# paganpasta/eqxvision

Measured on AMD Instinct MI355X. Metric: images/sec, higher is better.
Workload: dtype bf16; 1 GPU; resnet50 bf16 forward, batch=256/GPU, 3x224x224, 1000 classes; global_batch=256, parallelism=dp1, graph=True, lanes=2, collective_forced_1rank=False

## Files before the change

### eqxvision_amd/_lib.py

```python
from __future__ import annotations

import ctypes as C
import os
import threading

from . import _trace

_HERE = os.path.dirname(os.path.abspath(__file__))
LIB_PATH = os.environ.get("EQV_LIB") or os.path.join(_HERE, "csrc", "libeqxvision_amd.so")

F32, BF16 = 0, 1
ACT_NONE, ACT_RELU, ACT_GELU_TANH = 0, 1, 2
ACT_HARD_SWISH, ACT_HARD_SIGMOID, ACT_SIGMOID, ACT_SILU = 3, 4, 5, 6
ABI_VERSION = 2

_vp, _i, _f, _i64 = C.c_void_p, C.c_int, C.c_float, C.c_int64

PROTOTYPES = {
    "mv_abi_version": [],
    "mv_last_error": [],
    "mv_last_kernel": [],
    "mv_set_flag": [C.c_char_p, _i],
    "mv_get_flag": [C.c_char_p],
    "mv_flags_epoch": [],
# ... 53 lines not shown
    "mv_cnblock_dw_fwd": [_vp, _vp, _vp, _vp, _i, _i, _i, _i, _f, _i, _i, _i, _vp],
    "mv_conv2d_nchw_split_fwd": [_vp, _vp, _vp, _vp, _vp, _vp] + [_i] * 11 + [_i, _i, _i, _vp],
    "mv_resize_bilinear_nhwc_fwd": [_vp, _vp] + [_i] * 6 + [_i, _i, _i, _vp],
    "mv_copy_rows": [_vp, _vp, _i64, _i64, _i64, _i64, _vp],
    "mv_maxpool2d_nhwc_fwd": [_vp, _vp] + [_i] * 10 + [_i, _vp],
    "mv_adaptive_avgpool2d_nhwc_fwd": [_vp, _vp] + [_i] * 6 + [_i, _i, _vp],
    "mv_layernorm_fwd": [_vp, _vp, _vp, _vp, _i64, _i, _i64, _f, _i, _i, _vp],
    "mv_mha_fwd": [_vp, _vp, _vp, _i, _i, _i, _i, _f, _i, _vp],
    "mv_stem_conv_pool_supported": [_i] * 14 + [_i64],
    "mv_stem_conv_pool_fwd": [_vp, _vp, _vp, _vp, _vp] + [_i] * 17 + [_vp],
    "mv_conv1x1_chain_supported": [_i64, _i, _i, _i, _i],
    "mv_conv1x1_chain_fwd": [_vp] * 10 + [_i64, _i, _i, _i, _i, _vp],
    "mv_bottleneck_tail_supported": [_i] * 5,
    "mv_bottleneck_tail_fwd": [_vp] * 9 + [_i] * 6 + [_vp],
    "mv_conv1x1_dual_supported": [_i64, _i, _i, _i, _i],
    "mv_conv1x1_dual_fwd": [_vp] * 6 + [_i] * 11 + [_vp],
    "mv_conv1x1_chain_res_supported": [_i] * 8,
    "mv_conv1x1_chain_res_fwd": [_vp] * 6 + [_i] * 8 + [_vp],
    "mv_conv1x1_chain_rc_supported": [_i64, _i, _i, _i, _i],
    "mv_conv1x1_chain_rc_fwd": [_vp] * 7 + [_i64, _i, _i, _i, _i, _vp],
    "mv_conv1x1_chain_rc0_fwd": [_vp] * 5 + [_i64, _i, _i, _i, _i, _vp],
    "mv_conv1x1_chain_sub_supported": [_i] * 7,
    "mv_conv1x1_chain_sub_fwd": [_vp] * 10 + [_i] * 7 + [_vp],
    "mv_conv1x1_dual_chain_supported": [_i64, _i, _i, _i, _i, _i],
    "mv_conv1x1_dual_chain_fwd": [_vp] * 10 + [_i64, _i, _i, _i, _i, _i, _vp],
    "mv_linear_heads_supported": [_i64, _i, _i, _i, _i, _i],
    "mv_linear_lnout_supported": [_i64, _i, _i, _i],
    "mv_linear_lnout_fwd": [_vp, _vp, _vp, _vp, _vp, _vp, _vp, _vp, _i64, _i, _i, _i, _vp],
    "mv_linear_lnin_supported": [_i64, _i, _i, _i, _i, _i],
    "mv_linear_lnin_fwd": [_vp, _vp, _vp, _vp, _vp, _vp, _i64, _i, _i, _f, _i, _i, _i, _i, _vp],
    "mv_linear_heads_fwd": [_vp, _vp, _vp, _vp, _vp, _i64, _i, _i, _i, _i, _i, _vp],
    "mv_mha_heads_fwd": [_vp, _vp, _vp, _i, _i, _i, _i, _f, _i, _vp],
    "mv_mha_dropout_fwd": [_vp, _i, _vp, _vp, _vp, _f, _i, _i, _i, _i, _f, _i, _vp],
    "mv_swin_window_attn_fwd": [_vp, _vp, _vp] + [_i] * 9 + [_i, _vp],
    "mv_patch_merge_gather_nhwc": [_vp, _vp, _i, _i, _i, _i, _i, _vp],
    "mv_patch4_ln_supported": [_i] * 5,
    "mv_patch4_ln_fwd": [_vp] * 7 + [_i] * 5 + [_f, _i, _vp],
    "mv_patch_merge_ln_supported": [_i] * 4,
    "mv_patch_merge_ln_fwd": [_vp, _vp, _vp, _vp, _i, _i, _i, _i, _f, _i, _i, _vp],
    "mv_vit_cls_pos_fwd": [_vp, _vp, _vp, _i, _i, _i, _i, _vp],
    "mv_eltwise_fwd": [_vp, _vp, _i64, _i, _i, _vp],
    "mv_add_fwd": [_vp, _vp, _vp, _i64, _i, _i, _vp],
    "mv_channel_affine_fwd": [_vp, _vp, _vp, _vp, _i64, _i, _i, _i, _vp],
    "mv_channel_affine_res_fwd": [_vp, _vp, _vp, _vp, _vp, _i64, _i, _i, _i, _vp],
    "mv_nchw_to_nhwc": [_vp, _vp, _i, _i, _i, _i, _i, _i, _vp],
    "mv_nhwc_to_nchw": [_vp, _vp, _i, _i, _i, _i, _i, _i, _vp],
# ... 153 lines not shown
```

### eqxvision_amd/csrc/chain_rc.hip

```cpp
#include "mfma_common.h"

namespace mv {

struct ChainRcP {
    const bf16_t* t2;
    const bf16_t* t2p;
    const bf16_t* x0;
    const bf16_t* wf;
    const unsigned* sh;
    bf16_t* y;
    bf16_t* t1;
    int M, tiles_m;
    int dbg;
};

typedef short s16x2 __attribute__((ext_vector_type(2)));
__device__ __forceinline__ uint32_t relu_pack_bf2(float a, float b) {
    uint32_t w = pack_bf2(a, b);
    asm volatile("" : "+v"(w));
    const s16x2 z = {0, 0};
    return __builtin_bit_cast(uint32_t, __builtin_elementwise_max(__builtin_bit_cast(s16x2, w), z));
}

template <int NPREV, int WAVES, int RD>
__global__ __launch_bounds__(WAVES * 64) void chain_rc_kernel(const ChainRcP p) {
    constexpr int K = 256, N2 = 64, FPC = 12 + 4 * NPREV, NFRAG = 8 * FPC, PITCH = 144, NSH = 8 * (1 + NPREV) + 2, NT = WAVES * 64,
                  NX = 8 + 4 * NPREV;
    extern __shared__ __attribute__((aligned(16))) char smem[];
    char* wl = smem;
    const int tid = threadIdx.x, lane = tid & 63, wave = tid >> 6;
    char* ep = smem + NFRAG * 1024 + NSH * 256 + wave * (32 * PITCH);

    {
        constexpr int N16 = NFRAG * 64, U = 4;
        for (int base = 0; base < N16; base += U * NT) {
            uint4 v[U];
#pragma unroll
            for (int u = 0; u < U; ++u) {
                const int i = base + u * NT + tid;
                v[u] = ((const uint4*)p.wf)[i < N16 ? i : N16 - 1];
            }
#pragma unroll
            for (int u = 0; u < U; ++u) {
                const int i = base + u * NT + tid;
                if (i < N16) ((uint4*)wl)[i] = v[u];
// ... 472 lines not shown
```

### eqxvision_amd/csrc/common.h

```cpp
#pragma once
#include <atomic>
#include <hip/hip_runtime.h>
#include <stdint.h>
#include <stdio.h>
#include <string.h>

#include "../../include/eqxvision_amd.h"

namespace mv {

typedef uint16_t bf16_t;

__device__ __forceinline__ float bf2f(bf16_t v) { return __uint_as_float(((uint32_t)v) << 16); }

typedef __bf16 bf16x2_t __attribute__((ext_vector_type(2)));
__device__ __forceinline__ bf16_t f2bf(float f) { return __builtin_bit_cast(bf16_t, (__bf16)f); }
__device__ __forceinline__ uint32_t pack_bf2(float lo, float hi) {
    bf16x2_t v;
    v[0] = (__bf16)lo;
    v[1] = (__bf16)hi;
    return __builtin_bit_cast(uint32_t, v);
}

template <typename T> struct io;
// ... 134 lines not shown
                  int dh, int dw, int act, int out_dtype, int m_end, int tok, hipStream_t stream);
int igemm2_tile_shape(long long M, int K, int* bm, int* bn);
int igemm2_dual_supported(long long M, int C1, int C2, int K, int dtype);
int igemm2_dual_launch(const void* x, const void* x2, const void* w, const float* scale, const float* shift, void* y, int N,
                       int Ho, int Wo, int C1, int H2, int W2, int C2, int s2, int K, int act, hipStream_t st);
void igemm2_force_tile(int tile);
int tile_override(const char* kind, long long M, int a, int b, int R, int S, int sh);
int chain1x1_supported(long long M, int C, int K, int N2, int dtype);
int chain1x1_dual_supported(long long M, int C1, int C2, int K, int N2, int dtype);
int chain1x1_dual_launch(const void* x, const void* x2, const void* wcat, const float* scale3, const float* shift3, void* y,
                         const void* w1, const float* scale1, const float* shift1, void* t1, long long M, hipStream_t st);
int chain1x1_launch(const void* x, const void* w3, const float* scale3, const float* shift3, const void* residual, void* y,
                    const void* w1, const float* scale1, const float* shift1, void* t1, long long M, int N2, hipStream_t st);
int chain1x1_sub_supported(long long N, int H, int W, int C, int K, int N2, int dtype);
int chain1x1_sub_launch(const void* x, const void* w3, const float* scale3, const float* shift3, const void* residual, void* y_sub,
                        const void* w1, const float* scale1, const float* shift1, void* t1, int N, int H, int W, hipStream_t st);
int chain_rc_supported(long long M, int C, int K, int N2, int dtype);
int chain_rc_launch(const void* t2, const void* t2_prev, const void* x0, const void* wfrag, const void* shifts, void* y, void* t1,
                    long long M, hipStream_t st);
int chain_rc0_launch(const void* t2, const void* x0, const void* wfrag, const void* shifts, void* t1, long long M, hipStream_t st);
int chain_res_supported(long long N, int H, int W, int C, int K, int N2, int sub, int dtype);
int chain_res_launch(const void* t2, const void* residual, const void* wfrag, const void* shifts, void* y, void* t1, int N, int H, int W,
                     int sub, hipStream_t st);
int chain_stream_supported(long long M, int C, int K, int N2, int dtype);
int chain_stream_launch(const void* x, const void* w3, const float* scale3, const float* shift3, const void* residual, void* y,
                        const void* w1, const float* scale1, const float* shift1, void* t1, long long M, hipStream_t st);
int igemm8_supported(long long M, int C, int K, int R, int S, long long x_bytes, long long w_bytes);
int device_status(int clear, unsigned* out);
int igemm8_wanted(long long M, int C, int K, int R, int S);
int igemm8_launch(const void* x, const void* w, const float* scale, const float* shift, const void* residual, void* y,
                  int N, int H, int W, int C, int K, int R, int S, int sh, int sw, int ph, int pw, int dh, int dw,
                  int act, int out_dtype, int tok, int tile, hipStream_t st);
bool igemm8_ln_supported(long long M, int N, int K);
int igemm8_lnout_launch(const void* x, const void* w, const float* shift, const void* res, const void* res_lo, void* y, void* y_lo,
                        float* stats, long long M, int N, int K, hipStream_t st);
int igemm8_lnin_launch(const void* x, const float* stats, const void* w, const float* colsum, const float* shift, void* y, long long M,
                       int N, int K, float eps, int act, int tok, hipStream_t st);
int igemm8_dual_launch(const void* x, const void* x2, const void* w, const float* scale, const float* shift,
                       const void* residual, void* y, int N, int Ho, int Wo, int C1, int H2, int W2, int C2, int s2, int K,
                       int act, int out_dtype, int tile, hipStream_t st);
int stem_supported(int C, int K, int R, int S, int x_dtype, int out_dtype);
int stem_f32out_supported(int C, int H, int W, int K, int R, int S, int sh, int sw, int ph, int pw, int x_dtype);
int stem_launch(const void* x, const void* w, const float* scale, const float* shift, void* y, int N, int C,
                int H, int W, int K, int R, int S, int sh, int sw, int ph, int pw, int act, int x_dtype,
                int out_dtype, int tok_stride, int tok_offset, const float* pos, hipStream_t stream,
                const void* w_lo = nullptr);
// ... 21 lines not shown
```

### eqxvision_amd/csrc/generic.hip

```cpp
#include "mfma_common.h"

namespace mv {

struct ConvP {
    int N, H, W, C, K, R, S, Ho, Wo, sh, sw, ph, pw, dh, dw, groups;
    long long sxn, sxc, sxh, sxw;
    long long swk, swc, swr, sws;
    int act, tok_stride, tok_offset;
};

template <typename TX, typename TW, typename TY>
__global__ void conv_generic_kernel(const TX* __restrict__ x, const TW* __restrict__ w,
                                    const float* __restrict__ scale, const float* __restrict__ shift,
                                    const TY* __restrict__ residual, TY* __restrict__ y,
                                    const float* __restrict__ pos, ConvP p) {
    const int k = blockIdx.y * blockDim.x + threadIdx.x;
    const long long m = (long long)blockIdx.x * blockDim.y + threadIdx.y;
    const long long M = (long long)p.N * p.Ho * p.Wo;
    if (k >= p.K || m >= M) return;
    const int wo = (int)(m % p.Wo);
    const int ho = (int)((m / p.Wo) % p.Ho);
    const int n = (int)(m / ((long long)p.Wo * p.Ho));
    const int Cg = p.C / p.groups, Kg = p.K / p.groups;
    const int g = k / Kg;
// ... 1217 lines not shown
    if (chain_stream_supported(M, C, K, N2, dtype))
        return chain_stream_launch(x, w3, scale3, shift3, residual, y, w1, scale1, shift1, t1, M, (hipStream_t)stream);
    return chain1x1_launch(x, w3, scale3, shift3, residual, y, w1, scale1, shift1, t1, M, N2, (hipStream_t)stream);
}

int mv_conv1x1_chain_sub_supported(int N, int H, int W, int C, int K, int N2, int dtype) {
    return !get_flag("force_generic") && !get_flag("no_stream") && N > 0 && H > 0 && W > 0 && chain1x1_sub_supported(N, H, W, C, K, N2, dtype);
}

int mv_conv1x1_chain_sub_fwd(const void* x, const void* w3, const float* scale3, const float* shift3, const void* residual,
                             void* y_sub, const void* w1, const float* scale1, const float* shift1, void* t1, int N, int H, int W,
                             int C, int K, int N2, int dtype, mv_stream_t stream) {
    MV_CHECK_ARG(x && w3 && residual && y_sub && w1 && t1, "conv1x1_chain_sub: NULL pointer");
    if (!mv_conv1x1_chain_sub_supported(N, H, W, C, K, N2, dtype)) {
        set_error("conv1x1_chain_sub: unsupported shape N=%d H=%d W=%d C=%d K=%d N2=%d (ask mv_conv1x1_chain_sub_supported first)", N, H,
                  W, C, K, N2);
        return MV_E_UNSUPPORTED;
    }
    MV_CHECK_ARG(y_sub != residual && y_sub != x && t1 != y_sub, "conv1x1_chain_sub: y_sub must not alias x / residual / t1");
    return chain1x1_sub_launch(x, w3, scale3, shift3, residual, y_sub, w1, scale1, shift1, t1, N, H, W, (hipStream_t)stream);
}

int mv_conv1x1_chain_res_supported(int N, int H, int W, int C, int K, int N2, int sub, int dtype) {
    return !get_flag("force_generic") && !get_flag("no_stream") && N > 0 && H > 0 && W > 0 && chain_res_supported(N, H, W, C, K, N2, sub, dtype);
}

int mv_conv1x1_chain_res_fwd(const void* t2, const void* residual, const void* wfrag, const void* shifts, void* y, void* t1, int N, int H,
                             int W, int C, int K, int N2, int sub, int dtype, mv_stream_t stream) {
    MV_CHECK_ARG(t2 && residual && wfrag && shifts && y && t1, "conv1x1_chain_res: NULL pointer");
    if (!mv_conv1x1_chain_res_supported(N, H, W, C, K, N2, sub, dtype)) {
        set_error("conv1x1_chain_res: unsupported shape N=%d H=%d W=%d C=%d K=%d N2=%d sub=%d (ask mv_conv1x1_chain_res_supported first)", N,
                  H, W, C, K, N2, sub);
        return MV_E_UNSUPPORTED;
    }
    MV_CHECK_ARG(y != residual && y != t2 && t1 != y && t1 != residual && t1 != t2, "conv1x1_chain_res: outputs must not alias inputs");
    return chain_res_launch(t2, residual, wfrag, shifts, y, t1, N, H, W, sub, (hipStream_t)stream);
}

int mv_conv1x1_chain_rc_supported(int64_t M, int C, int K, int N2, int dtype) {
    return !get_flag("force_generic") && !get_flag("no_stream") && chain_rc_supported(M, C, K, N2, dtype);
}

int mv_conv1x1_chain_rc_fwd(const void* t2, const void* t2_prev, const void* x0, const void* wfrag, const void* shifts, void* y,
                            void* t1, int64_t M, int C, int K, int N2, int dtype, mv_stream_t stream) {
    MV_CHECK_ARG(t2 && t2_prev && x0 && wfrag && shifts && y && t1, "conv1x1_chain_rc: NULL pointer");
    if (!mv_conv1x1_chain_rc_supported(M, C, K, N2, dtype)) {
        set_error("conv1x1_chain_rc: unsupported shape M=%lld C=%d K=%d N2=%d (ask mv_conv1x1_chain_rc_supported first)", (long long)M, C,
                  K, N2);
        return MV_E_UNSUPPORTED;
    }
    MV_CHECK_ARG(y != t2 && y != t2_prev && y != x0 && t1 != y && t1 != t2 && t1 != t2_prev && t1 != x0,
                 "conv1x1_chain_rc: outputs must not alias inputs");
    return chain_rc_launch(t2, t2_prev, x0, wfrag, shifts, y, t1, M, (hipStream_t)stream);
}

int mv_conv1x1_chain_rc0_fwd(const void* t2, const void* x0, const void* wfrag, const void* shifts, void* t1, int64_t M, int C, int K,
                             int N2, int dtype, mv_stream_t stream) {
    MV_CHECK_ARG(t2 && x0 && wfrag && shifts && t1, "conv1x1_chain_rc0: NULL pointer");
    if (!mv_conv1x1_chain_rc_supported(M, C, K, N2, dtype)) {
// ... 752 lines not shown
```

### eqxvision_amd/csrc/mfma_common.h

```cpp
#pragma once
#include "common.h"

namespace mv {

typedef __bf16 bf16x8 __attribute__((ext_vector_type(8)));
typedef float f32x16 __attribute__((ext_vector_type(16)));

__device__ __forceinline__ void glds16(const void* gsrc, void* lds_dst) {
    __builtin_amdgcn_global_load_lds((const __attribute__((address_space(1))) void*)gsrc,
                                     (__attribute__((address_space(3))) void*)lds_dst, 16, 0, 0);
}

__device__ __forceinline__ void wave_lds_fence() {
    __builtin_amdgcn_fence(__ATOMIC_RELEASE, "wavefront");
    __builtin_amdgcn_wave_barrier();
    __builtin_amdgcn_fence(__ATOMIC_ACQUIRE, "wavefront");
}

typedef __amdgpu_buffer_rsrc_t brsrc_t;
typedef unsigned int u32x4_t __attribute__((ext_vector_type(4)));
constexpr unsigned BUF_OOB = 0x80000000u;

__device__ __forceinline__ brsrc_t make_brsrc(const void* base, bool live = true) {
    return __builtin_amdgcn_make_buffer_rsrc((void*)base, (short)0, live ? (int)BUF_OOB : 0, 0x00020000);
}
__device__ __forceinline__ float4 buf_load_f4(brsrc_t r, unsigned vo, unsigned so = 0) {
    const u32x4_t u = __builtin_amdgcn_raw_buffer_load_b128(r, vo, so, 0);
    return make_float4(__uint_as_float(u[0]), __uint_as_float(u[1]), __uint_as_float(u[2]), __uint_as_float(u[3]));
}
__device__ __forceinline__ void buf_store_f4(brsrc_t r, unsigned vo, float4 v) {
    u32x4_t u;
    u[0] = __float_as_uint(v.x); u[1] = __float_as_uint(v.y); u[2] = __float_as_uint(v.z); u[3] = __float_as_uint(v.w);
    __builtin_amdgcn_raw_buffer_store_b128(u, r, vo, 0, 0);
}
__device__ __forceinline__ uint4 buf_load_u4(brsrc_t r, unsigned vo, unsigned so = 0) {
    const u32x4_t u = __builtin_amdgcn_raw_buffer_load_b128(r, vo, so, 0);
    return make_uint4(u[0], u[1], u[2], u[3]);
}
__device__ __forceinline__ void buf_store_u4(brsrc_t r, unsigned vo, uint4 v) {
// ... 83 lines not shown
```

### eqxvision_amd/ops.py

```python
from __future__ import annotations

from typing import Optional, Tuple

import numpy as np
import torch

from . import _lib
from ._act import (Act, is_act, DT, TORCH_DT, compute_dtype, device, empty, head_fp32, on_replay, residual_fp32, split_weights,
                   stream_ptr)

ACT = {None: _lib.ACT_NONE, "none": _lib.ACT_NONE, "relu": _lib.ACT_RELU, "gelu": _lib.ACT_GELU_TANH,
       "hard_swish": _lib.ACT_HARD_SWISH, "hard_sigmoid": _lib.ACT_HARD_SIGMOID, "sigmoid": _lib.ACT_SIGMOID, "silu": _lib.ACT_SILU}
UNFUSED_ACTS = ("hard_swish", "hard_sigmoid", "sigmoid", "silu")


def _ptr(t: Optional[torch.Tensor]):
    return None if t is None else t.data_ptr()


def _dev(a: np.ndarray, dtype: torch.dtype) -> torch.Tensor:
    a = np.ascontiguousarray(a)
    if dtype == torch.bfloat16 and a.dtype == np.float32 and a.size < (1 << 20):
        u = a.view(np.uint32)
        r = ((u >> np.uint32(16)) & np.uint32(1)) + np.uint32(0x7FFF)
# ... 356 lines not shown
    y = empty((B, Ho, Wo, K), torch.bfloat16)
    _lib.call("mv_copy_rows", _ptr(yp), _ptr(y), B * Ho * Wo, K * 2, Kp * 2, K * 2, stream_ptr())
    return Act(y, "map", x.batched)


def _pointwise(conv) -> bool:
    return (tuple(conv.kernel_size) == (1, 1) and tuple(conv.stride) == (1, 1) and tuple(conv.padding) == (0, 0)
            and tuple(conv.dilation) == (1, 1) and conv.groups == 1)


def conv1x1_chain(x: Act, conv3, bn3, residual: Act, conv1n, bn1n, sub: int = 0) -> Optional[Act]:
    dt = compute_dtype()
    if dt != "bf16" or not (_pointwise(conv3) and _pointwise(conv1n)) or conv3.out_channels != conv1n.in_channels:
        return None
    if _bn_training(bn3) or _bn_training(bn1n):
        return None
    x, residual = as_map(x), as_map(residual)
    B, H, W, C = x.t.shape
    K, N2 = conv3.out_channels, conv1n.out_channels
    M = B * H * W
    if C != conv3.in_channels or tuple(residual.t.shape) != (B, H, W, K) or x.t.dtype != torch.bfloat16 \
            or residual.t.dtype != torch.bfloat16:
        return None
    if not _lib.load().mv_conv1x1_chain_supported(M, C, K, N2, DT[dt]):
        return None
    lib = _lib.load()
    for sb in ((2, 0) if sub == 2 else (0,)):
        if lib.mv_conv1x1_chain_res_supported(B, H, W, C, K, N2, sb, DT[dt]):
            wf, shf, _ = chain_res_fragments(conv3, bn3, conv1n, bn1n)
            y = empty((B, H // 2, W // 2, K) if sb else (B, H, W, K), torch.bfloat16)
            t1 = empty((B, H, W, N2), torch.bfloat16)
            _lib.call("mv_conv1x1_chain_res_fwd", _ptr(x.t), _ptr(residual.t), _ptr(wf), _ptr(shf), _ptr(y), _ptr(t1), B, H, W, C, K, N2,
                      sb, DT[dt], stream_ptr())
            out = Act(y, "map", x.batched)
            out.sub = 2 if sb else None
            out.pre = (conv1n, Act(t1, "map", x.batched))
            return out
    w3, s3, h3 = prep_conv(conv3, bn3, "krsc", dt)
    w1, s1, h1 = prep_conv(conv1n, bn1n, "krsc", dt)
    t1 = empty((B, H, W, N2), torch.bfloat16)
    if sub == 2 and _lib.load().mv_conv1x1_chain_sub_supported(B, H, W, C, K, N2, DT[dt]):
        y = empty((B, H // 2, W // 2, K), torch.bfloat16)
        _lib.call("mv_conv1x1_chain_sub_fwd", _ptr(x.t), _ptr(w3), _ptr(s3), _ptr(h3), _ptr(residual.t), _ptr(y), _ptr(w1), _ptr(s1),
                  _ptr(h1), _ptr(t1), B, H, W, C, K, N2, DT[dt], stream_ptr())
        out = Act(y, "map", x.batched)
        out.sub = 2
    else:
        y = empty((B, H, W, K), torch.bfloat16)
        _lib.call("mv_conv1x1_chain_fwd", _ptr(x.t), _ptr(w3), _ptr(s3), _ptr(h3), _ptr(residual.t), _ptr(y), _ptr(w1), _ptr(s1),
                  _ptr(h1), _ptr(t1), M, C, K, N2, DT[dt], stream_ptr())
        out = Act(y, "map", x.batched)
    out.pre = (conv1n, Act(t1, "map", x.batched))
    return out


def _rc_shift_rows(*vecs) -> np.ndarray:
    rows = []
    for v in vecs:
        v = np.asarray(v, np.float32).reshape(-1, 32)
        hi = torch.from_numpy(v).to(torch.bfloat16)
# ... 27 lines not shown
        frags = np.empty((K // 32, 16, 2, 32, 8), np.float32)
        e8 = np.arange(8)
        for c in range(K // 32):
            rows = slice(32 * c, 32 * c + 32)
            for fh in range(2):
                for kk in range(8):
                    frags[c, kk, fh] = wcat[rows][:, 16 * kk + 8 * fh + e8]
                for kk in range(4):
                    frags[c, 8 + kk, fh] = w31[rows][:, 16 * kk + 8 * fh + e8]
            _rc_conv1n_frags(frags, 12, w1n, c)
        sh = _rc_shift_rows(h30 + hd, h1, hn)
        hit = (_dev(frags.reshape(-1), torch.bfloat16), torch.from_numpy(sh.view(np.int32)).to(device()), (conv3_0, ds_conv, conv1n))
        cache[key] = hit
    return hit


def chain_res_fragments(conv3, bn3, conv1n, bn1n):
    cache = conv3._cache()
    key = ("chain_res", _bn_id(bn3), id(conv1n), _bn_id(bn1n))
    hit = cache.get(key)
    if hit is None:
        w3, h3 = _scaled_rows(conv3, bn3)
        w1n, hn = _scaled_rows(conv1n, bn1n)
        K, T2 = w3.shape[0], w1n.shape[0] // 32
        frags = np.empty((K // 32, 4 + 2 * T2, 2, 32, 8), np.float32)
        e8 = np.arange(8)
        for c in range(K // 32):
            rows = slice(32 * c, 32 * c + 32)
            for fh in range(2):
                for kk in range(4):
                    frags[c, kk, fh] = w3[rows][:, 16 * kk + 8 * fh + e8]
                for s_ in range(2):
                    cols = 32 * c + 16 * s_ + 4 * fh + np.array([0, 1, 2, 3, 8, 9, 10, 11])
                    for a2 in range(T2):
                        frags[c, 4 + T2 * s_ + a2, fh] = w1n[32 * a2:32 * a2 + 32][:, cols]
        sh = _rc_shift_rows(h3, hn)
        hit = (_dev(frags.reshape(-1), torch.bfloat16), torch.from_numpy(sh.view(np.int32)).to(device()), conv1n)
        cache[key] = hit
    return hit


def chain_rc0_fragments(conv3_0, bn3_0, ds_conv, ds_bn, conv1n, bn1n):
    cache = conv3_0._cache()
    key = ("chain_rc0", _bn_id(bn3_0), id(ds_conv), _bn_id(ds_bn), id(conv1n), _bn_id(bn1n))
    hit = cache.get(key)
    if hit is None:
        w30, h30 = _scaled_rows(conv3_0, bn3_0)
        wd, hd = _scaled_rows(ds_conv, ds_bn)
        wcat = np.concatenate([w30, wd], axis=1)
        w1n, hn = _scaled_rows(conv1n, bn1n)
        K = wcat.shape[0]
        frags = np.empty((K // 32, 12, 2, 32, 8), np.float32)
        e8 = np.arange(8)
        for c in range(K // 32):
            rows = slice(32 * c, 32 * c + 32)
            for fh in range(2):
                for kk in range(8):
                    frags[c, kk, fh] = wcat[rows][:, 16 * kk + 8 * fh + e8]
            _rc_conv1n_frags(frags, 8, w1n, c)
        sh = _rc_shift_rows(h30 + hd, hn)
# ... 142 lines not shown


def chain_rc_available(x: Act, b0, cd, b1, b2) -> bool:
    if compute_dtype() != "bf16" or _lib.get_flag("no_chain_rc"):
        return False
    convs = (b0.conv3, cd[0], b1.conv1, b1.conv3, b2.conv1)
    if not all(_pointwise(c) for c in convs) or any(_bn_training(b) for b in (b0.bn1, b0.bn2, b0.bn3, cd[1], b1.bn1, b1.bn2, b1.bn3, b2.bn1)):
        return False
    if x.kind != "map" or x.t.dtype != torch.bfloat16:
        return False
    B, H, W, C = x.t.shape
    M, K = B * H * W, b0.conv3.out_channels
    if b0.conv3.in_channels != C or cd[0].in_channels != C or b1.conv3.in_channels != C or cd[0].out_channels != K \
            or b1.conv3.out_channels != K or b1.conv1.in_channels != K or b2.conv1.in_channels != K \
            or tuple(b0.conv2.stride) != (1, 1) or tuple(b1.conv2.stride) != (1, 1) or b0.conv2.out_channels != C or b1.conv2.out_channels != C:
        return False
    lib = _lib.load()
    return bool(lib.mv_conv1x1_dual_chain_supported(M, C, C, K, b1.conv1.out_channels, DT["bf16"])
                and lib.mv_conv1x1_chain_rc_supported(M, C, K, b2.conv1.out_channels, DT["bf16"]))


def conv1x1_dual_chain(x: Act, conv3, bn3, xin: Act, ds_conv, ds_bn, conv1n, bn1n, store_y: bool = True) -> Optional[Act]:
    dt = compute_dtype()
    if dt != "bf16" or not (_pointwise(conv3) and _pointwise(ds_conv) and _pointwise(conv1n)):
        return None
    if conv3.out_channels != ds_conv.out_channels or conv3.out_channels != conv1n.in_channels:
        return None
    if any(_bn_training(b) for b in (bn3, ds_bn, bn1n)):
        return None
    x, xin = as_map(x), as_map(xin)
    B, H, W, C1 = x.t.shape
    C2, K, N2 = xin.t.shape[-1], conv3.out_channels, conv1n.out_channels
    M = B * H * W
    if tuple(xin.t.shape[:3]) != (B, H, W) or C1 != conv3.in_channels or C2 != ds_conv.in_channels \
            or x.t.dtype != torch.bfloat16 or xin.t.dtype != torch.bfloat16:
        return None
    if not _lib.load().mv_conv1x1_dual_chain_supported(M, C1, C2, K, N2, DT[dt]):
        return None
    if not store_y and not _lib.get_flag("no_chain_rc0") and _lib.load().mv_conv1x1_chain_rc_supported(M, C1, K, N2, DT[dt]):
        wf, tab, _ = chain_rc0_fragments(conv3, bn3, ds_conv, ds_bn, conv1n, bn1n)
        t1 = empty((B, H, W, N2), torch.bfloat16)
        _lib.call("mv_conv1x1_chain_rc0_fwd", _ptr(x.t), _ptr(xin.t), _ptr(wf), _ptr(tab), _ptr(t1), M, C1, K, N2, DT[dt], stream_ptr())
        return Act(t1, "map", x.batched)
    wcat, shift = _dual_weights(conv3, bn3, ds_conv, ds_bn)
    w1, s1, h1 = prep_conv(conv1n, bn1n, "krsc", dt)
    y = empty((B, H, W, K), torch.bfloat16) if store_y else None
    t1 = empty((B, H, W, N2), torch.bfloat16)
    _lib.call("mv_conv1x1_dual_chain_fwd", _ptr(x.t), _ptr(xin.t), _ptr(wcat), None, _ptr(shift), _ptr(y), _ptr(w1), _ptr(s1),
              _ptr(h1), _ptr(t1), M, C1, C2, K, N2, DT[dt], stream_ptr())
    if not store_y:
        return Act(t1, "map", x.batched)
    out = Act(y, "map", x.batched)
    out.pre = (conv1n, Act(t1, "map", x.batched))
    return out


def stem_conv_pool(x: Act, conv, bn, act, pool) -> Act:
    if _bn_training(bn):
        return maxpool2d(conv2d(x, conv, bn, act), pool.kernel_size, pool.stride, pool.padding)
    dt = compute_dtype()
# ... 953 lines not shown
```

### include/eqxvision_amd.h

```cpp
#ifndef EQXVISION_AMD_H
#define EQXVISION_AMD_H

#include <stddef.h>
#include <stdint.h>

#ifdef __cplusplus
extern "C" {
#endif

#define MV_ABI_VERSION 2

typedef void* mv_stream_t;

enum { MV_F32 = 0, MV_BF16 = 1 };
enum { MV_ACT_NONE = 0, MV_ACT_RELU = 1, MV_ACT_GELU_TANH = 2, MV_ACT_HARD_SWISH = 3, MV_ACT_HARD_SIGMOID = 4, MV_ACT_SIGMOID = 5,
       MV_ACT_SILU = 6 };
enum { MV_OK = 0, MV_E_INVALID = -1, MV_E_UNSUPPORTED = -2, MV_E_OOM = -3 };

int mv_abi_version(void);
const char* mv_last_error(void);
int mv_set_flag(const char* name, int value);
int mv_get_flag(const char* name);
int mv_flags_epoch(void);
int mv_device_status(int clear, unsigned* status);
// ... 28 lines not shown
                         const void* residual, void* y, const void* w1, const float* scale1,
                         const float* shift1, void* t1, int64_t M, int C, int K, int N2, int dtype,
                         mv_stream_t stream);

int mv_bottleneck_tail_supported(int H, int W, int width, int cout, int dtype);
int mv_bottleneck_tail_fwd(const void* t1, const void* w2f, const float* scale2, const float* shift2, const void* w3f,
                           const float* scale3, const float* shift3, const void* residual, void* y, int B, int H, int W,
                           int width, int cout, int dtype, mv_stream_t stream);

int mv_conv1x1_dual_supported(int64_t M, int C1, int C2, int K, int dtype);
int mv_conv1x1_dual_fwd(const void* x, const void* x2, const void* wcat, const float* scale, const float* shift,
                        void* y, int N, int Ho, int Wo, int C1, int H2, int W2, int C2, int stride2, int K,
                        int act, int dtype, mv_stream_t stream);

int mv_conv1x1_dual_chain_supported(int64_t M, int C1, int C2, int K, int N2, int dtype);
int mv_conv1x1_dual_chain_fwd(const void* x, const void* x2, const void* wcat, const float* scale,
                              const float* shift, void* y, const void* w1, const float* scale1,
                              const float* shift1, void* t1, int64_t M, int C1, int C2, int K, int N2,
                              int dtype, mv_stream_t stream);

int mv_conv1x1_chain_res_supported(int N, int H, int W, int C, int K, int N2, int sub, int dtype);
int mv_conv1x1_chain_res_fwd(const void* t2, const void* residual, const void* wfrag, const void* shifts, void* y, void* t1, int N, int H,
                             int W, int C, int K, int N2, int sub, int dtype, mv_stream_t stream);
int mv_conv1x1_chain_rc_supported(int64_t M, int C, int K, int N2, int dtype);
int mv_conv1x1_chain_rc0_fwd(const void* t2, const void* x0, const void* wfrag, const void* shifts, void* t1, int64_t M, int C, int K,
                             int N2, int dtype, mv_stream_t stream);
int mv_conv1x1_chain_rc_fwd(const void* t2, const void* t2_prev, const void* x0, const void* wfrag, const void* shifts, void* y,
                            void* t1, int64_t M, int C, int K, int N2, int dtype, mv_stream_t stream);
int mv_conv1x1_chain_sub_supported(int N, int H, int W, int C, int K, int N2, int dtype);
int mv_conv1x1_chain_sub_fwd(const void* x, const void* w3, const float* scale3, const float* shift3, const void* residual,
                             void* y_sub, const void* w1, const float* scale1, const float* shift1, void* t1, int N, int H, int W,
                             int C, int K, int N2, int dtype, mv_stream_t stream);

int mv_linear_fwd(const void* x, const void* w, const float* scale, const float* shift,
                  const void* residual, void* y, int64_t M, int N, int K,
                  int act, int in_dtype, int out_dtype, mv_stream_t stream);

int mv_linear_split_supported(int64_t M, int N, int K, int dtype);
int mv_linear_split_fwd(const void* x, const void* w_hi_lo, const float* scale, const float* shift, const void* residual,
                        void* y, int64_t M, int N, int K, int act, int in_dtype, int out_dtype, mv_stream_t stream);
int mv_conv2d_nchw_split_fwd(const void* x, const void* w_hi, const void* w_lo, const float* scale, const float* shift,
                             void* y, int N, int C, int H, int W, int K, int R, int S, int sh, int sw, int ph, int pw,
                             int act, int x_dtype, int out_dtype, mv_stream_t stream);

int mv_channel_scale_nhwc_fwd(const void* x, const void* s, void* y, int N, int64_t HW, int C, int dtype, mv_stream_t stream);

// ... 197 lines not shown
```

Baseline: 84690 images/s.

## Add fused layer2 chain kernels for residual and dual-downsample bottleneck transitions

```diff
diff --git a/eqxvision_amd/_lib.py b/eqxvision_amd/_lib.py
--- a/eqxvision_amd/_lib.py
+++ b/eqxvision_amd/_lib.py
@@ -99,6 +99,8 @@
     "mv_conv1x1_chain_rc0_fwd": [_vp] * 5 + [_i64, _i, _i, _i, _i, _vp],
     "mv_conv1x1_chain_sub_supported": [_i] * 7,
     "mv_conv1x1_chain_sub_fwd": [_vp] * 10 + [_i] * 7 + [_vp],
+    "mv_conv1x1_dual_chain_res_supported": [_i64, _i, _i, _i, _i, _i],
+    "mv_conv1x1_dual_chain_res_fwd": [_vp] * 6 + [_i64, _i, _i, _i, _i, _i, _vp],
     "mv_conv1x1_dual_chain_supported": [_i64, _i, _i, _i, _i, _i],
     "mv_conv1x1_dual_chain_fwd": [_vp] * 10 + [_i64, _i, _i, _i, _i, _i, _vp],
     "mv_linear_heads_supported": [_i64, _i, _i, _i, _i, _i],
diff --git a/eqxvision_amd/csrc/chain_l2.hip b/eqxvision_amd/csrc/chain_l2.hip
--- /dev/null
+++ b/eqxvision_amd/csrc/chain_l2.hip
@@ -0,0 +1,312 @@
+#include <type_traits>
+#include "mfma_common.h"
+
+namespace mv {
+
+struct ChainL2P {
+    const bf16_t* xa;
+    const bf16_t* xb;
+    const bf16_t* res;
+    const bf16_t* wf;
+    const unsigned* sh;
+    bf16_t* y;
+    bf16_t* t1;
+    int M, tiles_m, subH, subW, rounds, act;
+};
+
+template <int C1, int C2, bool RES, int N2, bool SUB, int WAVES, int AHEAD, int RD>
+__global__ __launch_bounds__(WAVES * 64) void chain_l2_kernel(const ChainL2P p) {
+    constexpr int K = 512, NCH = K / 32, KA = C1 / 16, KX = (C1 + C2) / 16, T2 = N2 / 32, FPC = KX + 2 * T2, CB = FPC * 1024,
+                  NSH = NCH + T2, NT = WAVES * 64, PT = FPC * 64 / NT, PITCH = 144;
+    static_assert((FPC * 64) % NT == 0 && RD <= FPC && (AHEAD == 1 || AHEAD == 2) && NCH % 2 == 0, "chain_l2 shape");
+    extern __shared__ __attribute__((aligned(16))) char smem[];
+    char* wbuf = smem;
+    unsigned* shl = (unsigned*)(smem + 2 * CB);
+    const int tid = threadIdx.x, lane = tid & 63, wave = tid >> 6;
+    char* ep = smem + 2 * CB + NSH * 256 + wave * (32 * PITCH);
+
+    auto wload = [&](int c, u32x4_t* wr) {
+        const u32x4_t* src = (const u32x4_t*)p.wf + c * (CB / 16);
+#pragma unroll
+        for (int u = 0; u < PT; ++u) wr[u] = src[u * NT + tid];
+    };
+    auto wstore = [&](int buf, const u32x4_t* wr) {
+#pragma unroll
+        for (int u = 0; u < PT; ++u) ((u32x4_t*)(wbuf + buf * CB))[u * NT + tid] = wr[u];
+    };
+    auto block_sync = [&]() {
+        asm volatile("s_waitcnt lgkmcnt(0)\n\ts_barrier" ::: "memory");
+        __builtin_amdgcn_sched_barrier(0);
+    };
+
+    u32x4_t wreg[AHEAD][PT];
+    wload(0, wreg[0]);
+    if constexpr (AHEAD == 2) wload(1, wreg[1]);
+    for (int i = tid; i < NSH * 64; i += NT) shl[i] = p.sh[i];
+    wstore(0, wreg[0]);
+    block_sync();
+
+    const int fr = lane & 31, fh = lane >> 5;
+    typedef __attribute__((address_space(3))) const char* lds_cp;
+    unsigned wb0 = (unsigned)(uintptr_t)(lds_cp)wbuf + lane * 16;
+    unsigned wb1 = wb0 + CB;
+    unsigned sbase = (unsigned)(uintptr_t)(lds_cp)(const char*)shl + lane * 4;
+    asm volatile("" : "+v"(wb0), "+v"(wb1), "+v"(sbase));
+    auto afrag = [&](int buf, int f) -> bf16x8 {
+        const lds_cp b = (lds_cp)(uintptr_t)(buf ? wb1 : wb0);
+        return __builtin_bit_cast(bf16x8, *(const __attribute__((address_space(3))) u32x4_t*)(b + f * 1024));
+    };
+    auto sfrag = [&](int row) -> bf16x8 {
+        u32x4_t v;
+        v[0] = *(const __attribute__((address_space(3))) unsigned*)((lds_cp)(uintptr_t)sbase + row * 256);
+        v[1] = 0u; v[2] = 0u; v[3] = 0u;
+        return __builtin_bit_cast(bf16x8, v);
+    };
+    u32x4_t onesv;
+    onesv[0] = fh ? 0u : 0x3f803f80u; onesv[1] = 0u; onesv[2] = 0u; onesv[3] = 0u;
+    const bf16x8 ones = __builtin_bit_cast(bf16x8, onesv);
+
+    auto load_x = [&](uint4* xf, int tile) {
+        int m = tile * 32 + fr;
+        m = m < p.M ? m : p.M - 1;
+#pragma unroll
+        for (int kk = 0; kk < KA; ++kk) xf[kk] = *(const uint4*)(p.xa + (long long)m * C1 + fh * 8 + kk * 16);
+#pragma unroll
+        for (int kk = 0; kk < KX - KA; ++kk) xf[KA + kk] = *(const uint4*)(p.xb + (long long)m * C2 + fh * 8 + kk * 16);
+    };
+    struct Rows2 { uint4 r0, r1; };
+    auto load_res = [&](int tile, int c) -> Rows2 {
+        Rows2 o;
+        if constexpr (RES) {
+            auto row = [&](int pass) -> uint4 {
+                int m = tile * 32 + pass * 16 + (lane >> 2);
+                m = m < p.M ? m : p.M - 1;
+                return *(const uint4*)(p.res + (long long)m * K + c * 32 + (lane & 3) * 8);
+            };
+            o.r0 = row(0); o.r1 = row(1);
+        } else {
+            o.r0 = make_uint4(0, 0, 0, 0); o.r1 = o.r0;
+        }
+        return o;
+    };
+
+    uint4 xf[KX];
+    const int tbase = p.tiles_m / (int)gridDim.x, trem = p.tiles_m % (int)gridDim.x;
+    const int nb = tbase + ((int)blockIdx.x < trem ? 1 : 0);
+    const int tile0 = (int)blockIdx.x * tbase + ((int)blockIdx.x < trem ? (int)blockIdx.x : trem);
+    const int wv = __builtin_amdgcn_readfirstlane(wave);
+    int tile = tile0 + wave;
+    load_x(xf, tile);
+    Rows2 rr = load_res(tile, 0);
+
+    for (int r = 0; r < p.rounds; ++r, tile += p.act) {
+        if (!(wv < p.act && r * p.act + wv < nb)) {
+#pragma unroll 1
+            for (int c0 = 0; c0 < NCH; c0 += 2)
+#pragma unroll
+                for (int ci = 0; ci < 2; ++ci) {
+                    const int c = c0 + ci, cn = c + AHEAD < NCH ? c + AHEAD : c + AHEAD - NCH;
+                    wload(cn, wreg[ci % AHEAD]);
+                    wstore(ci ^ 1, wreg[(ci + 1) % AHEAD]);
+                    block_sync();
+                }
+            continue;
+        }
+        const int tile_u = __builtin_amdgcn_readfirstlane(tile);
+        const int ntile = tile + p.act;
+        const brsrc_t ry = SUB ? make_brsrc(p.y) : make_brsrc(p.y + (long long)tile_u * 32 * K);
+        const brsrc_t rt = make_brsrc(p.t1 + (long long)tile_u * 32 * N2);
+        const int rows_left = p.M - tile_u * 32;
+        unsigned yoff[2];
+#pragma unroll
+        for (int pass = 0; pass < 2; ++pass) {
+            const int row = pass * 16 + (lane >> 2);
+            if constexpr (SUB) {
+                const int m = tile_u * 32 + row, hw = p.subH * p.subW;
+                const int b = m / hw, rem = m - b * hw;
+                const int h = rem / p.subW, w = rem - h * p.subW;
+                yoff[pass] = m < p.M && !((h | w) & 1) ? (unsigned)(((b * (p.subH >> 1) + (h >> 1)) * (p.subW >> 1) + (w >> 1)) * K) * 2u
+                                                       : BUF_OOB;
+            } else {
+                yoff[pass] = row < rows_left ? (unsigned)(row * K) * 2u : BUF_OOB;
+            }
+        }
+        f32x16 acc2[T2];
+#pragma unroll
+        for (int a2 = 0; a2 < T2; ++a2) {
+            f32x16 z;
+#pragma unroll
+            for (int e = 0; e < 16; ++e) z[e] = 0.f;
+            acc2[a2] = __builtin_amdgcn_mfma_f32_32x32x16_bf16(sfrag(NCH + a2), ones, z, 0, 0, 0);
+        }
+
+        auto step = [&](auto CI, const int c, auto LAST) {
+            constexpr int ci = decltype(CI)::value;
+            {
+                const int cn = c + AHEAD < NCH ? c + AHEAD : c + AHEAD - NCH;
+                wload(cn, wreg[ci % AHEAD]);
+            }
+            bf16x8 ring[RD];
+#pragma unroll
+            for (int d = 0; d < RD; ++d) ring[d] = afrag(ci, d);
+            auto take = [&](int i) -> bf16x8 {
+                __builtin_amdgcn_sched_barrier(0);
+                const bf16x8 a = ring[i % RD];
+                if (i + RD < FPC) ring[i % RD] = afrag(ci, i + RD);
+                return a;
+            };
+            f32x16 a;
+            if constexpr (RES) {
+                {
+                    char* w = ep + (lane >> 2) * PITCH + (lane & 3) * 16;
+                    *(uint4*)(w) = rr.r0; *(uint4*)(w + 16 * PITCH) = rr.r1;
+                }
+                wave_lds_fence();
+                rr = load_res(c + 1 < NCH ? tile : ntile, c + 1 < NCH ? c + 1 : 0);
+#pragma unroll
+                for (int g = 0; g < 4; ++g) {
+                    const uint2 u = *(const uint2*)(ep + fr * PITCH + (8 * g + 4 * fh) * 2);
+                    a[4 * g] = __uint_as_float(u.x << 16);
+                    a[4 * g + 1] = __uint_as_float(u.x & 0xffff0000u);
+                    a[4 * g + 2] = __uint_as_float(u.y << 16);
+                    a[4 * g + 3] = __uint_as_float(u.y & 0xffff0000u);
+                }
+                wave_lds_fence();
+            } else {
+#pragma unroll
+                for (int e = 0; e < 16; ++e) a[e] = 0.f;
+            }
+            a = __builtin_amdgcn_mfma_f32_32x32x16_bf16(sfrag(c), ones, a, 0, 0, 0);
+#pragma unroll
+            for (int kk = 0; kk < KX; ++kk) {
+                const bf16x8 af = take(kk);
+                a = __builtin_amdgcn_mfma_f32_32x32x16_bf16(af, __builtin_bit_cast(bf16x8, xf[kk]), a, 0, 0, 0);
+                __builtin_amdgcn_sched_barrier(0);
+            }
+            uint32_t pk[8];
+#pragma unroll
+            for (int g = 0; g < 4; ++g) {
+                pk[2 * g] = relu_pack_bf2(a[4 * g], a[4 * g + 1]);
+                pk[2 * g + 1] = relu_pack_bf2(a[4 * g + 2], a[4 * g + 3]);
+                *(uint2*)(ep + fr * PITCH + (8 * g + 4 * fh) * 2) = make_uint2(pk[2 * g], pk[2 * g + 1]);
+            }
+            if constexpr (decltype(LAST)::value) load_x(xf, ntile);
+#pragma unroll
+            for (int q = 0; q < 2 * T2; ++q) {
+                const bf16x8 af = take(KX + q);
+                const int s = q / T2, a2 = q % T2;
+                const uint4 b = make_uint4(pk[4 * s], pk[4 * s + 1], pk[4 * s + 2], pk[4 * s + 3]);
+                acc2[a2] = __builtin_amdgcn_mfma_f32_32x32x16_bf16(af, __builtin_bit_cast(bf16x8, b), acc2[a2], 0, 0, 0);
+                __builtin_amdgcn_sched_barrier(0);
+            }
+            wave_lds_fence();
+#pragma unroll
+            for (int pass = 0; pass < 2; ++pass) {
+                const int row = pass * 16 + (lane >> 2);
+                const uint4 u = *(const uint4*)(ep + row * PITCH + (lane & 3) * 16);
+                buf_store_u4(ry, yoff[pass] == BUF_OOB ? BUF_OOB : yoff[pass] + (unsigned)(c * 32 + (lane & 3) * 8) * 2u, u);
+            }
+            wave_lds_fence();
+            wstore(ci ^ 1, wreg[(ci + 1) % AHEAD]);
+            block_sync();
+        };
+#pragma unroll 1
+        for (int c0 = 0; c0 < NCH - 2; c0 += 2) {
+            step(std::integral_constant<int, 0>(), c0, std::false_type());
+            step(std::integral_constant<int, 1>(), c0 + 1, std::false_type());
+        }
+        step(std::integral_constant<int, 0>(), NCH - 2, std::false_type());
+        step(std::integral_constant<int, 1>(), NCH - 1, std::true_type());
+
+#pragma unroll
+        for (int rd = 0; rd < T2 / 2; ++rd) {
+#pragma unroll
+            for (int a2 = 0; a2 < 2; ++a2)
+#pragma unroll
+                for (int g = 0; g < 4; ++g)
+                    *(uint2*)(ep + fr * PITCH + (a2 * 32 + 8 * g + 4 * fh) * 2) =
+                        make_uint2(relu_pack_bf2(acc2[2 * rd + a2][4 * g], acc2[2 * rd + a2][4 * g + 1]),
+                                   relu_pack_bf2(acc2[2 * rd + a2][4 * g + 2], acc2[2 * rd + a2][4 * g + 3]));
+            wave_lds_fence();
+#pragma unroll
+            for (int pass = 0; pass < 4; ++pass) {
+                const int row = pass * 8 + (lane >> 3);
+                const uint4 u = *(const uint4*)(ep + row * PITCH + (lane & 7) * 16);
+                buf_store_u4(rt, row < rows_left ? (unsigned)(row * N2 + rd * 64 + (lane & 7) * 8) * 2u : BUF_OOB, u);
+            }
+            wave_lds_fence();
+        }
+    }
+}
+
+template <int C1, int C2, bool RES, int N2, bool SUB, int WAVES, int AHEAD, int RD>
+static int chain_l2_go(ChainL2P& p, long long M, hipStream_t st) {
+    constexpr int FPC = (C1 + C2) / 16 + N2 / 16;
+    constexpr int SMEM = 2 * FPC * 1024 + (16 + N2 / 32) * 256 + WAVES * 32 * 144;
+    static_assert(SMEM <= 160 * 1024, "LDS");
+    p.M = (int)M;
+    p.tiles_m = (int)((M + 31) / 32);
+    int gx = 256;
+    const int need = (p.tiles_m + WAVES - 1) / WAVES;
+    if (gx > need) gx = need;
+    const int per_block = (p.tiles_m + gx - 1) / gx;
+    p.rounds = (per_block + WAVES - 1) / WAVES;
+    p.act = (per_block + p.rounds - 1) / p.rounds;
+    auto kern = chain_l2_kernel<C1, C2, RES, N2, SUB, WAVES, AHEAD, RD>;
+    static LdsAttrSite attr;
+    MV_HIP(attr.ensure((const void*)kern, SMEM));
+    hipLaunchKernelGGL(kern, dim3(gx), dim3(WAVES * 64), SMEM, st, p);
+    MV_LAUNCH_CHECK();
+    return MV_OK;
+}
+
+static bool chain_l2_m_ok(long long M) { return M >= 16384 && M < (1LL << 31) - (1 << 20); }
+
+int chain_l2_res_supported(long long N, int H, int W, int C, int K, int N2, int sub, int dtype) {
+    const long long M = N * H * W;
+    if (!(dtype == MV_BF16 && C == 128 && K == 512 && (N2 == 128 || N2 == 256) && chain_l2_m_ok(M)) || get_flag("no_chain") ||
+        get_flag("no_chain_res") || get_flag("no_chain_l2"))
+        return 0;
+    if (sub == 0) return 1;
+    return sub == 2 && H % 2 == 0 && W % 2 == 0 && N * (H / 2) * (W / 2) * K * 2 < (1LL << 31) && !get_flag("no_chain_sub");
+}
+
+int chain_l2_res_launch(const void* t2, const void* residual, const void* wfrag, const void* shifts, void* y, void* t1, int N, int H,
+                        int W, int N2, int sub, hipStream_t st) {
+    ChainL2P p;
+    p.xa = (const bf16_t*)t2; p.xb = nullptr; p.res = (const bf16_t*)residual; p.wf = (const bf16_t*)wfrag;
+    p.sh = (const unsigned*)shifts; p.y = (bf16_t*)y; p.t1 = (bf16_t*)t1;
+    p.subH = H; p.subW = W;
+    const long long M = (long long)N * H * W;
+    if (N2 == 256) {
+        if (sub) {
+            set_kernel_name("chain_l2_exit_bf16_128_512_256_ysub2");
+            return chain_l2_go<128, 0, true, 256, true, 4, 2, 6>(p, M, st);
+        }
+        set_kernel_name("chain_l2_exit_bf16_128_512_256");
+        return chain_l2_go<128, 0, true, 256, false, 4, 2, 6>(p, M, st);
+    }
+    if (sub) {
+        set_kernel_name("chain_l2_res_bf16_128_512_128_ysub2");
+        return chain_l2_go<128, 0, true, 128, true, 8, 2, 6>(p, M, st);
+    }
+    set_kernel_name("chain_l2_res_bf16_128_512_128");
+    return chain_l2_go<128, 0, true, 128, false, 8, 2, 6>(p, M, st);
+}
+
+int chain_l2_dual_supported(long long M, int C1, int C2, int K, int N2, int dtype) {
+    return dtype == MV_BF16 && C1 == 128 && C2 == 256 && K == 512 && N2 == 128 && chain_l2_m_ok(M) && !get_flag("no_chain") &&
+           !get_flag("no_chain_l2");
+}
+
+int chain_l2_dual_launch(const void* t2, const void* x, const void* wfrag, const void* shifts, void* y, void* t1, long long M,
+                         hipStream_t st) {
+    ChainL2P p;
+    p.xa = (const bf16_t*)t2; p.xb = (const bf16_t*)x; p.res = nullptr; p.wf = (const bf16_t*)wfrag;
+    p.sh = (const unsigned*)shifts; p.y = (bf16_t*)y; p.t1 = (bf16_t*)t1;
+    p.subH = 0; p.subW = 0;
+    set_kernel_name("chain_l2_entry_bf16_128+256_512_128");
+    return chain_l2_go<128, 256, false, 128, false, 4, 2, 6>(p, M, st);
+}
+
+}
diff --git a/eqxvision_amd/csrc/chain_rc.hip b/eqxvision_amd/csrc/chain_rc.hip
--- a/eqxvision_amd/csrc/chain_rc.hip
+++ b/eqxvision_amd/csrc/chain_rc.hip
@@ -13,14 +13,6 @@
     int M, tiles_m;
     int dbg;
 };
-
-typedef short s16x2 __attribute__((ext_vector_type(2)));
-__device__ __forceinline__ uint32_t relu_pack_bf2(float a, float b) {
-    uint32_t w = pack_bf2(a, b);
-    asm volatile("" : "+v"(w));
-    const s16x2 z = {0, 0};
-    return __builtin_bit_cast(uint32_t, __builtin_elementwise_max(__builtin_bit_cast(s16x2, w), z));
-}
 
 template <int NPREV, int WAVES, int RD>
 __global__ __launch_bounds__(WAVES * 64) void chain_rc_kernel(const ChainRcP p) {
diff --git a/eqxvision_amd/csrc/common.h b/eqxvision_amd/csrc/common.h
--- a/eqxvision_amd/csrc/common.h
+++ b/eqxvision_amd/csrc/common.h
@@ -180,6 +180,12 @@
 int chain_res_supported(long long N, int H, int W, int C, int K, int N2, int sub, int dtype);
 int chain_res_launch(const void* t2, const void* residual, const void* wfrag, const void* shifts, void* y, void* t1, int N, int H, int W,
                      int sub, hipStream_t st);
+int chain_l2_res_supported(long long N, int H, int W, int C, int K, int N2, int sub, int dtype);
+int chain_l2_res_launch(const void* t2, const void* residual, const void* wfrag, const void* shifts, void* y, void* t1, int N, int H,
+                        int W, int N2, int sub, hipStream_t st);
+int chain_l2_dual_supported(long long M, int C1, int C2, int K, int N2, int dtype);
+int chain_l2_dual_launch(const void* t2, const void* x, const void* wfrag, const void* shifts, void* y, void* t1, long long M,
+                         hipStream_t st);
 int chain_stream_supported(long long M, int C, int K, int N2, int dtype);
 int chain_stream_launch(const void* x, const void* w3, const float* scale3, const float* shift3, const void* residual, void* y,
                         const void* w1, const float* scale1, const float* shift1, void* t1, long long M, hipStream_t st);
diff --git a/eqxvision_amd/csrc/generic.hip b/eqxvision_amd/csrc/generic.hip
--- a/eqxvision_amd/csrc/generic.hip
+++ b/eqxvision_amd/csrc/generic.hip
@@ -1263,7 +1263,8 @@
 }
 
 int mv_conv1x1_chain_res_supported(int N, int H, int W, int C, int K, int N2, int sub, int dtype) {
-    return !get_flag("force_generic") && !get_flag("no_stream") && N > 0 && H > 0 && W > 0 && chain_res_supported(N, H, W, C, K, N2, sub, dtype);
+    return !get_flag("force_generic") && !get_flag("no_stream") && N > 0 && H > 0 && W > 0 &&
+           (chain_res_supported(N, H, W, C, K, N2, sub, dtype) || chain_l2_res_supported(N, H, W, C, K, N2, sub, dtype));
 }
 
 int mv_conv1x1_chain_res_fwd(const void* t2, const void* residual, const void* wfrag, const void* shifts, void* y, void* t1, int N, int H,
@@ -1275,7 +1276,25 @@
         return MV_E_UNSUPPORTED;
     }
     MV_CHECK_ARG(y != residual && y != t2 && t1 != y && t1 != residual && t1 != t2, "conv1x1_chain_res: outputs must not alias inputs");
+    if (C == 128)
+        return chain_l2_res_launch(t2, residual, wfrag, shifts, y, t1, N, H, W, N2, sub, (hipStream_t)stream);
     return chain_res_launch(t2, residual, wfrag, shifts, y, t1, N, H, W, sub, (hipStream_t)stream);
+}
+
+int mv_conv1x1_dual_chain_res_supported(int64_t M, int C1, int C2, int K, int N2, int dtype) {
+    return !get_flag("force_generic") && !get_flag("no_stream") && chain_l2_dual_supported(M, C1, C2, K, N2, dtype);
+}
+
+int mv_conv1x1_dual_chain_res_fwd(const void* t2, const void* x, const void* wfrag, const void* shifts, void* y, void* t1, int64_t M,
+                                  int C1, int C2, int K, int N2, int dtype, mv_stream_t stream) {
+    MV_CHECK_ARG(t2 && x && wfrag && shifts && y && t1, "conv1x1_dual_chain_res: NULL pointer");
+    if (!mv_conv1x1_dual_chain_res_supported(M, C1, C2, K, N2, dtype)) {
+        set_error("conv1x1_dual_chain_res: unsupported shape M=%lld C1=%d C2=%d K=%d N2=%d (ask mv_conv1x1_dual_chain_res_supported first)",
+                  (long long)M, C1, C2, K, N2);
+        return MV_E_UNSUPPORTED;
+    }
+    MV_CHECK_ARG(y != t2 && y != x && t1 != y && t1 != t2 && t1 != x, "conv1x1_dual_chain_res: outputs must not alias inputs");
+    return chain_l2_dual_launch(t2, x, wfrag, shifts, y, t1, M, (hipStream_t)stream);
 }
 
 int mv_conv1x1_chain_rc_supported(int64_t M, int C, int K, int N2, int dtype) {
diff --git a/eqxvision_amd/csrc/mfma_common.h b/eqxvision_amd/csrc/mfma_common.h
--- a/eqxvision_amd/csrc/mfma_common.h
+++ b/eqxvision_amd/csrc/mfma_common.h
@@ -15,6 +15,14 @@
     __builtin_amdgcn_fence(__ATOMIC_RELEASE, "wavefront");
     __builtin_amdgcn_wave_barrier();
     __builtin_amdgcn_fence(__ATOMIC_ACQUIRE, "wavefront");
+}
+
+typedef short s16x2 __attribute__((ext_vector_type(2)));
+__device__ __forceinline__ uint32_t relu_pack_bf2(float a, float b) {
+    uint32_t w = pack_bf2(a, b);
+    asm volatile("" : "+v"(w));
+    const s16x2 z = {0, 0};
+    return __builtin_bit_cast(uint32_t, __builtin_elementwise_max(__builtin_bit_cast(s16x2, w), z));
 }
 
 typedef __amdgpu_buffer_rsrc_t brsrc_t;
diff --git a/eqxvision_amd/ops.py b/eqxvision_amd/ops.py
--- a/eqxvision_amd/ops.py
+++ b/eqxvision_amd/ops.py
@@ -402,8 +402,6 @@
     if C != conv3.in_channels or tuple(residual.t.shape) != (B, H, W, K) or x.t.dtype != torch.bfloat16 \
             or residual.t.dtype != torch.bfloat16:
         return None
-    if not _lib.load().mv_conv1x1_chain_supported(M, C, K, N2, DT[dt]):
-        return None
     lib = _lib.load()
     for sb in ((2, 0) if sub == 2 else (0,)):
         if lib.mv_conv1x1_chain_res_supported(B, H, W, C, K, N2, sb, DT[dt]):
@@ -416,6 +414,8 @@
             out.sub = 2 if sb else None
             out.pre = (conv1n, Act(t1, "map", x.batched))
             return out
+    if not lib.mv_conv1x1_chain_supported(M, C, K, N2, DT[dt]):
+        return None
     w3, s3, h3 = prep_conv(conv3, bn3, "krsc", dt)
     w1, s1, h1 = prep_conv(conv1n, bn1n, "krsc", dt)
     t1 = empty((B, H, W, N2), torch.bfloat16)
@@ -489,20 +489,39 @@
     if hit is None:
         w3, h3 = _scaled_rows(conv3, bn3)
         w1n, hn = _scaled_rows(conv1n, bn1n)
-        K, T2 = w3.shape[0], w1n.shape[0] // 32
-        frags = np.empty((K // 32, 4 + 2 * T2, 2, 32, 8), np.float32)
-        e8 = np.arange(8)
-        for c in range(K // 32):
-            rows = slice(32 * c, 32 * c + 32)
-            for fh in range(2):
-                for kk in range(4):
-                    frags[c, kk, fh] = w3[rows][:, 16 * kk + 8 * fh + e8]
-                for s_ in range(2):
-                    cols = 32 * c + 16 * s_ + 4 * fh + np.array([0, 1, 2, 3, 8, 9, 10, 11])
-                    for a2 in range(T2):
-                        frags[c, 4 + T2 * s_ + a2, fh] = w1n[32 * a2:32 * a2 + 32][:, cols]
         sh = _rc_shift_rows(h3, hn)
-        hit = (_dev(frags.reshape(-1), torch.bfloat16), torch.from_numpy(sh.view(np.int32)).to(device()), conv1n)
+        hit = (_dev(_res_fragments(w3, w1n).reshape(-1), torch.bfloat16), torch.from_numpy(sh.view(np.int32)).to(device()), conv1n)
+        cache[key] = hit
+    return hit
+
+
+def _res_fragments(w3, w1n) -> np.ndarray:
+    K, KX, T2 = w3.shape[0], w3.shape[1] // 16, w1n.shape[0] // 32
+    frags = np.empty((K // 32, KX + 2 * T2, 2, 32, 8), np.float32)
+    e8 = np.arange(8)
+    for c in range(K // 32):
+        rows = slice(32 * c, 32 * c + 32)
+        for fh in range(2):
+            for kk in range(KX):
+                frags[c, kk, fh] = w3[rows][:, 16 * kk + 8 * fh + e8]
+            for s_ in range(2):
+                cols = 32 * c + 16 * s_ + 4 * fh + np.array([0, 1, 2, 3, 8, 9, 10, 11])
+                for a2 in range(T2):
+                    frags[c, KX + T2 * s_ + a2, fh] = w1n[32 * a2:32 * a2 + 32][:, cols]
+    return frags
+
+
+def chain_l2_dual_fragments(conv3, bn3, ds_conv, ds_bn, conv1n, bn1n):
+    cache = conv3._cache()
+    key = ("chain_l2_dual", _bn_id(bn3), id(ds_conv), _bn_id(ds_bn), id(conv1n), _bn_id(bn1n))
+    hit = cache.get(key)
+    if hit is None:
+        w3, h3 = _scaled_rows(conv3, bn3)
+        wd, hd = _scaled_rows(ds_conv, ds_bn)
+        w1n, hn = _scaled_rows(conv1n, bn1n)
+        frags = _res_fragments(np.concatenate([w3, wd], axis=1), w1n)
+        sh = _rc_shift_rows(h3 + hd, hn)
+        hit = (_dev(frags.reshape(-1), torch.bfloat16), torch.from_numpy(sh.view(np.int32)).to(device()), (ds_conv, conv1n))
         cache[key] = hit
     return hit
 
@@ -691,7 +710,8 @@
 
 def conv1x1_dual_chain(x: Act, conv3, bn3, xin: Act, ds_conv, ds_bn, conv1n, bn1n, store_y: bool = True) -> Optional[Act]:
     dt = compute_dtype()
-    if dt != "bf16" or not (_pointwise(conv3) and _pointwise(ds_conv) and _pointwise(conv1n)):
+    if dt != "bf16" or not (_pointwise(conv3) and _pointwise(conv1n)) or tuple(ds_conv.kernel_size) != (1, 1) \
+            or tuple(ds_conv.padding) != (0, 0) or tuple(ds_conv.dilation) != (1, 1) or ds_conv.groups != 1:
         return None
     if conv3.out_channels != ds_conv.out_channels or conv3.out_channels != conv1n.in_channels:
         return None
@@ -704,7 +724,18 @@
     if tuple(xin.t.shape[:3]) != (B, H, W) or C1 != conv3.in_channels or C2 != ds_conv.in_channels \
             or x.t.dtype != torch.bfloat16 or xin.t.dtype != torch.bfloat16:
         return None
-    if not _lib.load().mv_conv1x1_dual_chain_supported(M, C1, C2, K, N2, DT[dt]):
+    ds_stride = tuple(ds_conv.stride)
+    if store_y and (ds_stride == (1, 1) or (xin.sub is not None and ds_stride == (xin.sub, xin.sub))) \
+            and _lib.load().mv_conv1x1_dual_chain_res_supported(M, C1, C2, K, N2, DT[dt]):
+        wf, tab, _ = chain_l2_dual_fragments(conv3, bn3, ds_conv, ds_bn, conv1n, bn1n)
+        y = empty((B, H, W, K), torch.bfloat16)
+        t1 = empty((B, H, W, N2), torch.bfloat16)
+        _lib.call("mv_conv1x1_dual_chain_res_fwd", _ptr(x.t), _ptr(xin.t), _ptr(wf), _ptr(tab), _ptr(y), _ptr(t1), M, C1, C2, K, N2,
+                  DT[dt], stream_ptr())
+        out = Act(y, "map", x.batched)
+        out.pre = (conv1n, Act(t1, "map", x.batched))
+        return out
+    if not _pointwise(ds_conv) or not _lib.load().mv_conv1x1_dual_chain_supported(M, C1, C2, K, N2, DT[dt]):
         return None
     if not store_y and not _lib.get_flag("no_chain_rc0") and _lib.load().mv_conv1x1_chain_rc_supported(M, C1, K, N2, DT[dt]):
         wf, tab, _ = chain_rc0_fragments(conv3, bn3, ds_conv, ds_bn, conv1n, bn1n)
diff --git a/include/eqxvision_amd.h b/include/eqxvision_amd.h
--- a/include/eqxvision_amd.h
+++ b/include/eqxvision_amd.h
@@ -74,6 +74,9 @@
 int mv_conv1x1_chain_res_supported(int N, int H, int W, int C, int K, int N2, int sub, int dtype);
 int mv_conv1x1_chain_res_fwd(const void* t2, const void* residual, const void* wfrag, const void* shifts, void* y, void* t1, int N, int H,
                              int W, int C, int K, int N2, int sub, int dtype, mv_stream_t stream);
+int mv_conv1x1_dual_chain_res_supported(int64_t M, int C1, int C2, int K, int N2, int dtype);
+int mv_conv1x1_dual_chain_res_fwd(const void* t2, const void* x, const void* wfrag, const void* shifts, void* y, void* t1, int64_t M,
+                                  int C1, int C2, int K, int N2, int dtype, mv_stream_t stream);
 int mv_conv1x1_chain_rc_supported(int64_t M, int C, int K, int N2, int dtype);
 int mv_conv1x1_chain_rc0_fwd(const void* t2, const void* x0, const void* wfrag, const void* shifts, void* t1, int64_t M, int C, int K,
                              int N2, int dtype, mv_stream_t stream);
```

After: 86260 images/s (median of 6 runs). 1.9% higher.
